# rdd0582/mri_superresolution

Measured on AMD Instinct MI355X. Metric: 2D MRI slices/sec (train fwd+bwd) 256×256 U-Net; PSNR/SSIM vs ref, higher is better.
Workload: dtype bf16; 1 GPU; UNetSuperRes base_filters=64 depth=4, 256x256 slices -> 512x512, batch=16/GPU bf16, L1+SSIM(0.4), train step fwd+bwd+Adam+SSIM metric; global_batch=16, parallelism=dp1

## Files before the change

include/mrisr.h:

```cpp
#ifndef MRISR_H
#define MRISR_H

#include <stddef.h>
#include <stdint.h>

#ifdef __cplusplus
extern "C" {
#endif

#define MRISR_OK 0
#define MRISR_E_ARG (-1)
#define MRISR_E_SHAPE (-2)
#define MRISR_E_DTYPE (-3)
#define MRISR_E_HIP (-4)
#define MRISR_E_UNSUPPORTED (-5)

#define MRISR_F32 0
#define MRISR_BF16 1
#define MRISR_F16 2

#define MRISR_SRC_RAW 0
#define MRISR_SRC_NORM 1
#define MRISR_SRC_RELU 2
#define MRISR_SP_NONE 0
// ... 112 lines not shown
                         const float* blend_alpha, void* g, float* red, float* alpha_slots, int N, int H, int W,
                         int C, int groups, void* stream);
int mrisr_act_bwd_finalize(const float* red, const float* gamma, const float* meanrstd, float* dgamma,
                           float* dbeta, float* coef, int N, int C, int groups, double count,
                           const float* alpha_slots, const float* alpha, float* dalpha, float alpha_sign, void* stream);
int mrisr_act_bwd_apply(int dtype, const void* x, const void* g, const float* coef, void* dx, int N,
                        int H, int W, int C, int out_mode, float* dbias, void* stream);
typedef struct mrisr_gn_bwd_fin {
    const float* red;
    const float* gamma;
    const float* meanrstd;
    float* dgamma;
    float* dbeta;
    const float* alpha_slots;
    const float* alpha;
    float* dalpha;
    double count;
    float alpha_sign;
    int32_t groups;
} mrisr_gn_bwd_fin;
int mrisr_act_bwd_apply_fused(int dtype, const void* x, const float* scale, const float* shift, int nconsumers,
                              const mrisr_consumer* consumers, const float* blend_alpha, const float* coef,
                              const mrisr_gn_bwd_fin* fin, void* dx, int N, int H, int W, int C, void* stream);
int mrisr_act_bwd_onepass_slots(void);
int mrisr_act_bwd_onepass_barrier_words(void);
int mrisr_act_bwd_onepass_ok(int dtype, int nconsumers, const mrisr_consumer* consumers, int N, int H, int W, int C);
int mrisr_act_bwd_onepass(int dtype, const void* x, const float* scale, const float* shift, const float* meanrstd,
                          int nconsumers, const mrisr_consumer* consumers, float* red, uint32_t* arrive,
                          const mrisr_gn_bwd_fin* fin, void* dx, int N, int H, int W, int C, void* stream);
int mrisr_act_bwd_apply_fused_unshuffle(int dtype, const void* x, const float* scale, const float* shift,
                                        const mrisr_consumer* consumer, const float* blend_alpha,
                                        const mrisr_gn_bwd_fin* fin, void* dx, float* dbias, int N, int H, int W, int C,
                                        void* stream);
int mrisr_channel_sum(int dtype, const void* x, float* out, size_t npix, int C, void* stream);
int mrisr_blend_alpha_grad(int dtype, const void* da, const void* x0, const float* scale0,
                           const float* shift0, const void* x1, const float* scale1,
                           const float* shift1, const float* alpha, float* dalpha, int N, int H,
                           int W, int C, void* stream);

int mrisr_head_forward(int dtype, const void* x, const float* scale, const float* shift,
                       const float* w, const float* b, float* out, int N, int H, int W, int C,
                       void* stream);
int mrisr_head_backward(int dtype, const void* x, const float* scale, const float* shift,
                        const float* w, const float* out, const float* dout, void* da, float* dw,
                        float* db, int N, int H, int W, int C, void* stream);
int mrisr_head_forward_multi(int dtype, const void* x, const float* scale, const float* shift,
                             const float* w, const float* b, float* out, int N, int H, int W, int C,
                             int K, void* stream);
int mrisr_head_backward_multi(int dtype, const void* x, const float* scale, const float* shift,
                              const float* w, const float* out, const float* dout, void* da,
                              float* dw, float* db, int N, int H, int W, int C, int K, void* stream);

int mrisr_ssim_l1_forward(const float* a, const float* b, double* sums, float* coef, int N, int H,
                          int W, float val_range, float sigma, void* stream);
int mrisr_ssim_l1_backward(const float* a, const float* b, const float* coef, const double* sums,
                           const float* gscale, float l1_w, float ssim_w, float* da, int N, int H,
                           int W, float sigma, void* stream);
int mrisr_ssim_l1_forward_win(const float* a, const float* b, double* sums, float* coef, int N, int H, int W,
                              float val_range, float sigma, int window_size, void* stream);
int mrisr_ssim_l1_backward_win(const float* a, const float* b, const float* coef, const double* sums,
                               const float* gscale, float l1_w, float ssim_w, float* da, int N, int H, int W,
                               float sigma, int window_size, void* stream);

int mrisr_loss_finalize(const double* sums, int N, int H, int W, float l1_w, float ssim_w, float* out,
                        void* stream);

// ... 89 lines not shown
```

mri_superresolution_amd/_lib.py:

```python
from __future__ import annotations

import ctypes as C
import os

from .tuning import TUNING

_HERE = os.path.dirname(os.path.abspath(__file__))
LIB_PATH = TUNING.lib_path or os.path.join(_HERE, "libmrisr.so")

F32, BF16, F16 = 0, 1, 2
SRC_RAW, SRC_NORM, SRC_RELU = 0, 1, 2
SP_NONE, SP_POOL2, SP_UP2, SP_HEAD = 0, 1, 2, 3
COMBINE_CONCAT, COMBINE_BLEND = 0, 1
OUT_PLAIN, OUT_PIXEL_SHUFFLE2 = 0, 1
UP2_BILINEAR, UP2_BICUBIC, UP2_SHARP_BILINEAR = 0, 1, 2
WINDOW_F32, WINDOW_I16 = 0, 1
RESAMPLE_LINEAR, RESAMPLE_CUBIC, RESAMPLE_AREA, RESAMPLE_LANCZOS4 = 1, 2, 3, 4
PACK_RING = 256
PACK_UPADJ = 512
STAT_SLOTS = 16

_vp, _fp, _dp, _i, _f, _d, _sz = C.c_void_p, C.c_void_p, C.c_void_p, C.c_int, C.c_float, C.c_double, C.c_size_t


class Src(C.Structure):
    _fields_ = [("ptr", _vp), ("scale", _fp), ("shift", _fp), ("C", C.c_int32), ("H", C.c_int32),
                ("W", C.c_int32), ("mode", C.c_int32), ("spatial", C.c_int32), ("off_y", C.c_int32),
                ("off_x", C.c_int32)]


class ConvDesc(C.Structure):
    _fields_ = [("dtype", C.c_int32), ("N", C.c_int32), ("H", C.c_int32), ("W", C.c_int32),
                ("Cin", C.c_int32), ("Cout", C.c_int32), ("ksize", C.c_int32), ("nsrc", C.c_int32),
                ("combine", C.c_int32), ("out_mode", C.c_int32), ("groups", C.c_int32),
                ("relu_out", C.c_int32), ("src", Src * 2), ("blend_alpha", _fp), ("wpacked", _vp),
                ("bias", _fp), ("out", _vp), ("stats", _dp), ("relu_mask", _vp), ("cu_limit", C.c_int32),
                ("reserved_", C.c_int32), ("wpacked_ring", _vp)]


class PackJob(C.Structure):
    _fields_ = [("w", _fp), ("packed", _vp), ("Cout", C.c_int32), ("Cin", C.c_int32), ("ksize", C.c_int32),
                ("transpose_flip", C.c_int32)]


class AugGeo(C.Structure):
    _fields_ = [("cos_a", C.c_float), ("sin_a", C.c_float), ("rotate", C.c_int32), ("flip", C.c_int32),
                ("fill", C.c_int32), ("brightness", C.c_float)]


class AugPhoto(C.Structure):
    _fields_ = [("contrast", C.c_float), ("mean", C.c_int32), ("noise_sigma", C.c_float), ("seed", C.c_uint32)]


class GnBwdFin(C.Structure):
    _fields_ = [("red", _fp), ("gamma", _fp), ("meanrstd", _fp), ("dgamma", _fp), ("dbeta", _fp),
                ("alpha_slots", _fp), ("alpha", _fp), ("dalpha", _fp), ("count", C.c_double),
                ("alpha_sign", C.c_float), ("groups", C.c_int32)]


class Consumer(C.Structure):
    _fields_ = [("da", _vp), ("C_total", C.c_int32), ("c_off", C.c_int32), ("H", C.c_int32),
                ("W", C.c_int32), ("spatial", C.c_int32), ("off_y", C.c_int32), ("off_x", C.c_int32),
                ("weight_mode", C.c_int32), ("head_out", _fp), ("head_w", _fp), ("head_part", _fp),
                ("head_dw", _fp), ("head_db", _fp)]


SIGNATURES = {
    "mrisr_last_error": (C.c_char_p, []),
    "mrisr_version": (_i, []),
    "mrisr_stat_slots": (_i, []),
    "mrisr_packed_weight_bytes": (_sz, [_i, _i, _i, _i]),
    "mrisr_conv_ring_bn": (_i, [_i, _i, _i, _i]),
    "mrisr_packed_weight_bytes_ring": (_sz, [_i, _i, _i, _i]),
    "mrisr_pack_weights": (_i, [_i, _fp, _i, _i, _i, _i, _vp, _vp]),
    "mrisr_pack_weights_batched": (_i, [_i, _vp, _i, _vp]),
    "mrisr_conv_forward": (_i, [C.POINTER(ConvDesc), _vp]),
    "mrisr_packed_weight_bytes_upadj": (_sz, [_i, _i, _i, _i]),
    "mrisr_conv_upadj": (_i, [C.POINTER(ConvDesc), _vp, _vp, _vp]),
    "mrisr_conv_variant": (_i, [C.POINTER(ConvDesc), _i, C.c_char_p, _sz]),
    "mrisr_conv_wgrad": (_i, [C.POINTER(ConvDesc), _vp, _fp, _fp, _sz, _vp]),
    "mrisr_conv_wgrad_workspace_floats": (_sz, [C.POINTER(ConvDesc)]),
    "mrisr_stem_forward": (_i, [_i, _fp, _fp, _vp, _dp, _i, _i, _i, _i, _i, _vp]),
    "mrisr_stem_wgrad": (_i, [_i, _fp, _vp, _fp, _i, _i, _i, _i, _vp]),
    "mrisr_stem_forward_multi": (_i, [_i, _fp, _fp, _vp, _dp, _i, _i, _i, _i, _i, _i, _vp]),
    "mrisr_stem_wgrad_multi": (_i, [_i, _fp, _vp, _fp, _i, _i, _i, _i, _i, _vp]),
    "mrisr_gn_finalize": (_i, [_dp, _fp, _fp, _fp, _fp, _fp, _i, _i, _i, _d, _f, _vp]),
    "mrisr_norm_pool2": (_i, [_i, _vp, _fp, _fp, _vp, _i, _i, _i, _i, _vp]),
    "mrisr_norm_upsample2": (_i, [_i, _vp, _fp, _fp, _vp, _i, _i, _i, _i, _vp]),
    "mrisr_norm_blend": (_i, [_i, _vp, _fp, _fp, _vp, _fp, _fp, _fp, _vp, _i, _i, _i, _i, _vp]),
    "mrisr_upsample2_stats": (_i, [_i, _vp, _vp, _dp, _i, _i, _i, _i, _i, _vp]),
    "mrisr_up_conv1x1_fused": (_i, [_i, _vp, _fp, _fp, _vp, _vp, _dp, _i, _i, _i, _i, _i, _i, _vp]),
    "mrisr_upsample2_adjoint": (_i, [_i, _vp, _vp, _i, _i, _i, _i, _vp]),
    "mrisr_act_bwd_reduce": (_i, [_i, _vp, _fp, _fp, _fp, _i, C.POINTER(Consumer), _fp, _vp, _fp, _fp, _i, _i, _i, _i, _i, _vp]),
    "mrisr_act_bwd_finalize": (_i, [_fp, _fp, _fp, _fp, _fp, _fp, _i, _i, _i, _d, _fp, _fp, _fp, _f, _vp]),
    "mrisr_act_bwd_apply": (_i, [_i, _vp, _vp, _fp, _vp, _i, _i, _i, _i, _i, _fp, _vp]),
    "mrisr_act_bwd_apply_fused": (_i, [_i, _vp, _fp, _fp, _i, C.POINTER(Consumer), _fp, _fp, C.POINTER(GnBwdFin), _vp, _i, _i,
                                       _i, _i, _vp]),
    "mrisr_act_bwd_onepass_slots": (_i, []),
    "mrisr_act_bwd_onepass_barrier_words": (_i, []),
    "mrisr_act_bwd_onepass_ok": (_i, [_i, _i, C.POINTER(Consumer), _i, _i, _i, _i]),
    "mrisr_act_bwd_onepass": (_i, [_i, _vp, _fp, _fp, _fp, _i, C.POINTER(Consumer), _fp, _vp, C.POINTER(GnBwdFin), _vp, _i, _i, _i,
                                   _i, _vp]),
    "mrisr_act_bwd_apply_fused_unshuffle": (_i, [_i, _vp, _fp, _fp, C.POINTER(Consumer), _fp, C.POINTER(GnBwdFin), _vp, _fp, _i,
                                                 _i, _i, _i, _vp]),
    "mrisr_channel_sum": (_i, [_i, _vp, _fp, _sz, _i, _vp]),
    "mrisr_blend_alpha_grad": (_i, [_i, _vp, _vp, _fp, _fp, _vp, _fp, _fp, _fp, _fp, _i, _i, _i, _i, _vp]),
    "mrisr_head_forward": (_i, [_i, _vp, _fp, _fp, _fp, _fp, _fp, _i, _i, _i, _i, _vp]),
    "mrisr_head_backward": (_i, [_i, _vp, _fp, _fp, _fp, _fp, _fp, _vp, _fp, _fp, _i, _i, _i, _i, _vp]),
    "mrisr_head_forward_multi": (_i, [_i, _vp, _fp, _fp, _fp, _fp, _fp, _i, _i, _i, _i, _i, _vp]),
    "mrisr_head_backward_multi": (_i, [_i, _vp, _fp, _fp, _fp, _fp, _fp, _vp, _fp, _fp, _i, _i, _i, _i, _i, _vp]),
    "mrisr_ssim_l1_forward": (_i, [_fp, _fp, _dp, _fp, _i, _i, _i, _f, _f, _vp]),
    "mrisr_ssim_l1_backward": (_i, [_fp, _fp, _fp, _dp, _fp, _f, _f, _fp, _i, _i, _i, _f, _vp]),
    "mrisr_ssim_l1_forward_win": (_i, [_fp, _fp, _dp, _fp, _i, _i, _i, _f, _f, _i, _vp]),
    "mrisr_ssim_l1_backward_win": (_i, [_fp, _fp, _fp, _dp, _fp, _f, _f, _fp, _i, _i, _i, _f, _i, _vp]),
    "mrisr_loss_finalize": (_i, [_dp, _i, _i, _i, _f, _f, _fp, _vp]),
    "mrisr_image_metrics": (_i, [_fp, _fp, _dp, _i, _i, _i, _f, _f, _i, _vp]),
    "mrisr_metrics_finalize": (_i, [_dp, _i, _i, _i, _f, _dp, _vp]),
    "mrisr_vgg_input_channels": (_i, []),
    "mrisr_vgg_input_forward": (_i, [_i, _fp, _vp, _sz, _vp]),
    "mrisr_vgg_input_backward": (_i, [_i, _vp, _fp, _f, _fp, _sz, _vp]),
    "mrisr_maxpool2_forward": (_i, [_i, _vp, _vp, _i, _i, _i, _i, _vp]),
    "mrisr_maxpool2_backward": (_i, [_i, _vp, _vp, _vp, _i, _i, _i, _i, _i, _vp]),
    "mrisr_feature_loss": (_i, [_i, _vp, _vp, _sz, _i, _dp, _fp, _vp, _i, _vp]),
    "mrisr_adam_step": (_i, [_fp, _fp, _fp, _fp, _sz, _f, _f, _f, _f, _f, _i, _f, _vp]),
    "mrisr_adam_step_amp": (_i, [_fp, _fp, _fp, _fp, _sz, _f, _f, _f, _f, _f, _vp, _f, _fp, _fp, _vp]),
    "mrisr_u8_histogram": (_i, [_vp, _sz, _i, _vp, _vp]),
    "mrisr_u8_percentile_normalise": (_i, [_vp, _vp, _sz, _i, _d, _d, _fp, _fp, _vp]),
    "mrisr_f32_to_u8": (_i, [_fp, _vp, _sz, _vp]),
    "mrisr_u8_upscale2": (_i, [_vp, _vp, _fp, _i, _i, _i, _i, _vp]),
    "mrisr_u8_to_unit_f32": (_i, [_vp, _fp, _sz, _vp]),
    "mrisr_augment_geo_u8": (_i, [_vp, _vp, _i, _i, _i, _vp, _dp, _vp]),
    "mrisr_augment_finish_u8": (_i, [_vp, _fp, _i, _sz, _vp, _dp, _vp]),
    "mrisr_cast": (_i, [_i, _vp, _i, _vp, _sz, _vp]),
    "mrisr_lowfield_dirichlet": (_i, [_i, _d, _fp, _fp]),
    "mrisr_lowfield_workspace_bytes": (_sz, [_i, _i, _i]),
    "mrisr_lowfield_simulate": (_i, [_vp, _i, _i, _i, _d, _fp, _fp, _fp, _fp, _f, _fp, _fp, _vp, _vp, _vp, _fp, _vp]),
    "mrisr_lowfield_dirichlet_any": (_i, [_i, _d, _fp, _fp]),
    "mrisr_lowfield_simulate_f32": (_i, [_fp, _i, _i, _i, _d, _fp, _fp, _fp, _fp, _f, _fp, _fp, _vp, _vp, _fp, _vp]),
    "mrisr_resample_taps": (_i, [_i, _i, _i, _i, _vp, _vp, _fp]),
    "mrisr_f32_resample_letterbox": (_i, [_fp, _i, _i, _i, _vp, _fp, _i, _i, _vp, _fp, _i, _i, _i, _i, _i, _i, _f, _i, _fp, _vp, _vp]),
    "mrisr_f32_percentile_workspace_bytes": (_sz, [_i]),
    "mrisr_f32_percentile_bounds": (_i, [_fp, _sz, _i, _d, _d, _fp, _vp, _vp]),
    "mrisr_f32_window_normalise": (_i, [_fp, _fp, _sz, _i, _fp, _vp]),
    "mrisr_f32_window_restore": (_i, [_fp, _fp, _sz, _i, _i, _vp, _vp]),
}

_lib = None
ABI_VERSION = 308


def load():
    global _lib
    if _lib is not None:
        return _lib
    if not os.path.exists(LIB_PATH):
        raise RuntimeError(
            f"{LIB_PATH} not found: the HIP kernel library is not built. Run "
            "`python -m mri_superresolution_amd.build` (needs hipcc); there is no CPU fallback.")
    lib = C.CDLL(LIB_PATH)
    missing = [name for name in SIGNATURES if not hasattr(lib, name)]
    if missing:
        raise RuntimeError(f"{LIB_PATH} lacks {len(missing)} symbol(s) of include/mrisr.h ({', '.join(missing[:4])}...): "
                           "header/library drift - rebuild with `python -m mri_superresolution_amd.build`")
    for name, (res, args) in SIGNATURES.items():
        fn = getattr(lib, name)
        fn.restype = res
        fn.argtypes = args
    if int(lib.mrisr_version()) != ABI_VERSION:
        raise RuntimeError(f"{LIB_PATH} is version {int(lib.mrisr_version())}, these bindings need {ABI_VERSION} (struct layouts "
                           "changed): rebuild with `python -m mri_superresolution_amd.build`")
    global STAT_SLOTS
    STAT_SLOTS = int(lib.mrisr_stat_slots())
    _lib = lib
    return lib


def check(rc: int, what: str = ""):
    if rc != 0:
        msg = load().mrisr_last_error().decode("utf-8", "replace")
        raise RuntimeError(f"libmrisr {what} failed ({rc}): {msg}")

# ... 38 lines not shown
```

mri_superresolution_amd/csrc/api.cpp:

```cpp
#include "common.h"
thread_local char g_mrisr_err[512] = "";
extern "C" const char* mrisr_last_error(void) { return g_mrisr_err; }
extern "C" int mrisr_version(void) { return 308; }
extern "C" int mrisr_stat_slots(void) { return MRISR_STAT_SLOTS; }
```

mri_superresolution_amd/csrc/norm.hip:

```cpp
#include "common.h"

__global__ void gn_finalize_kernel(const double* __restrict__ stats, const float* __restrict__ gamma,
                                   const float* __restrict__ beta, float* __restrict__ scale,
                                   float* __restrict__ shift, float* __restrict__ meanrstd, int N, int C,
                                   int groups, double count, float eps) {
    const int idx = blockIdx.x * blockDim.x + threadIdx.x;
    if (idx >= N * C) return;
    const int n = idx / C, c = idx - n * C;
    const int gs = C / groups, g = c / gs;
    typedef __attribute__((ext_vector_type(2))) double f64x2;
    f64x2 v[MRISR_STAT_SLOTS];
#pragma unroll
    for (int k = 0; k < MRISR_STAT_SLOTS; ++k) v[k] = *reinterpret_cast<const f64x2*>(stats + ((size_t)(k * N + n) * groups + g) * 2);
    double s = 0.0, ss = 0.0;
#pragma unroll
    for (int k = 0; k < MRISR_STAT_SLOTS; ++k) { s += v[k][0]; ss += v[k][1]; }
    const double mean = s / count;
    double var = ss / count - mean * mean;
    if (var < 0) var = 0;
    const float rstd = (float)(1.0 / sqrt(var + (double)eps));
    const float m = (float)mean;
    const float sc = gamma[c] * rstd;
    scale[idx] = sc;
    shift[idx] = beta[c] - m * sc;
// ... 1179 lines not shown
                                                   const mrisr_gn_bwd_fin* fin, void* dx, float* dbias, int N, int H, int W,
                                                   int C, void* stream) {
    if (!x || !scale || !shift || !dx || !consumer || !fin) MRISR_FAIL(MRISR_E_ARG, "act_bwd_apply_fused_unshuffle: null pointer");
    if (!fin->red || !fin->gamma || !fin->meanrstd || !fin->dgamma || !fin->dbeta) MRISR_FAIL(MRISR_E_ARG, "act_bwd_apply_fused_unshuffle: fin null pointer");
    if (fin->groups <= 0 || fin->groups > kMaxGroups || C % fin->groups || !(fin->count > 0)) MRISR_FAIL(MRISR_E_SHAPE, "act_bwd_apply_fused_unshuffle: fin groups %d", fin->groups);
    if (fin->alpha_slots && (!fin->alpha || !fin->dalpha)) MRISR_FAIL(MRISR_E_ARG, "act_bwd_apply_fused_unshuffle: alpha_slots without alpha/dalpha");
    const int vec = mrisr_vec(dtype);
    if (C % vec || ((H | W) & 1)) MRISR_FAIL(MRISR_E_SHAPE, "act_bwd_apply_fused_unshuffle: C %d, H %d, W %d (even dims)", C, H, W);
    if (consumer->spatial != MRISR_SP_NONE || consumer->H != H || consumer->W != W || consumer->off_y || consumer->off_x)
        MRISR_FAIL(MRISR_E_UNSUPPORTED, "act_bwd_apply_fused_unshuffle: one plain consumer with the node's geometry");
    ActBwdParams p;
    memset(&p, 0, sizeof(p));
    p.x = x; p.scale = scale; p.shift = shift; p.blend_alpha = blend_alpha;
    p.ncons = 1; p.N = N; p.H = H; p.W = W; p.C = C;
    int rc = fill_act_bwd_params(p, dtype, 1, consumer, blend_alpha, H, W, C, "act_bwd_apply_fused_unshuffle");
    if (rc) return rc;
    const FinDev fd{fin->red, fin->gamma, fin->meanrstd, fin->dgamma, fin->dbeta, fin->alpha_slots, fin->alpha, fin->dalpha,
                    (float)(1.0 / fin->count), fin->alpha_sign, fin->groups, nullptr, nullptr, nullptr};
    const int nslice = ceil_div(C / vec, 256), nvs = nslice > 1 ? 256 : C / vec;
    const int ppbw = 256 / nvs, HWp = (H / 2) * (W / 2);
    int ppw = ppbw * 16;
    if (ppw > HWp) ppw = ceil_div(HWp, ppbw) * ppbw;
    p.pix_per_block = ppw;
    dim3 grid(ceil_div(HWp, ppw), N, nslice);
    hipStream_t s = (hipStream_t)stream;
    if (dtype == MRISR_BF16) act_bwd_unshuffle_window_kernel<bf16_t><<<grid, 256, 0, s>>>(p, (bf16_t*)dx, dbias, fd);
    else if (dtype == MRISR_F16) act_bwd_unshuffle_window_kernel<f16_t><<<grid, 256, 0, s>>>(p, (f16_t*)dx, dbias, fd);
    else if (dtype == MRISR_F32) act_bwd_unshuffle_window_kernel<float><<<grid, 256, 0, s>>>(p, (float*)dx, dbias, fd);
    else MRISR_FAIL(MRISR_E_DTYPE, "act_bwd_apply_fused_unshuffle: dtype %d", dtype);
    MRISR_CHECK_LAUNCH("act_bwd_apply_fused_unshuffle");
    return MRISR_OK;
}

extern "C" int mrisr_act_bwd_apply(int dtype, const void* x, const void* g, const float* coef, void* dx, int N, int H,
                                   int W, int C, int out_mode, float* dbias, void* stream) {
    if (!x || !g || !coef || !dx) MRISR_FAIL(MRISR_E_ARG, "act_bwd_apply: null pointer");
    const int vec = mrisr_vec(dtype);
    if (C % vec) MRISR_FAIL(MRISR_E_SHAPE, "act_bwd_apply: C %d", C);
    if (out_mode == MRISR_OUT_PIXEL_SHUFFLE2 && ((H | W) & 1)) MRISR_FAIL(MRISR_E_SHAPE, "act_bwd_apply: odd dims with pixel shuffle");
    const size_t total = (size_t)N * H * W * (C / vec);
    const int blocks = (int)((total + 255) / 256 < 8192 ? (total + 255) / 256 : 8192);
    if (dbias && !(out_mode == MRISR_OUT_PIXEL_SHUFFLE2 && (4 * C) % vec == 0 && 256 % (4 * C / vec) == 0))
        MRISR_FAIL(MRISR_E_UNSUPPORTED, "act_bwd_apply: dbias needs the pixel-shuffle output with 4C/vec dividing 256");
    if (out_mode == MRISR_OUT_PIXEL_SHUFFLE2 && (4 * C) % vec == 0) {
        const int blocks = dbias ? (int)((total + 255) / 256 < 1024 ? (total + 255) / 256 : 1024) : (int)((total + 255) / 256 < 8192 ? (total + 255) / 256 : 8192);
        if (dtype == MRISR_BF16)
            act_bwd_apply_unshuffle_kernel<bf16_t><<<blocks, 256, 0, (hipStream_t)stream>>>((const bf16_t*)x, (const bf16_t*)g, coef, (bf16_t*)dx, N, H, W, C, dbias);
        else if (dtype == MRISR_F16)
            act_bwd_apply_unshuffle_kernel<f16_t><<<blocks, 256, 0, (hipStream_t)stream>>>((const f16_t*)x, (const f16_t*)g, coef, (f16_t*)dx, N, H, W, C, dbias);
        else if (dtype == MRISR_F32)
            act_bwd_apply_unshuffle_kernel<float><<<blocks, 256, 0, (hipStream_t)stream>>>((const float*)x, (const float*)g, coef, (float*)dx, N, H, W, C, dbias);
        else MRISR_FAIL(MRISR_E_DTYPE, "act_bwd_apply: dtype %d", dtype);
        MRISR_CHECK_LAUNCH("act_bwd_apply");
        return MRISR_OK;
    }
    if (dtype == MRISR_BF16)
        act_bwd_apply_kernel<bf16_t><<<blocks, 256, 0, (hipStream_t)stream>>>((const bf16_t*)x, (const bf16_t*)g, coef, (bf16_t*)dx, N, H, W, C, out_mode);
    else if (dtype == MRISR_F16)
        act_bwd_apply_kernel<f16_t><<<blocks, 256, 0, (hipStream_t)stream>>>((const f16_t*)x, (const f16_t*)g, coef, (f16_t*)dx, N, H, W, C, out_mode);
    else if (dtype == MRISR_F32)
        act_bwd_apply_kernel<float><<<blocks, 256, 0, (hipStream_t)stream>>>((const float*)x, (const float*)g, coef, (float*)dx, N, H, W, C, out_mode);
    else MRISR_FAIL(MRISR_E_DTYPE, "act_bwd_apply: dtype %d", dtype);
    MRISR_CHECK_LAUNCH("act_bwd_apply");
    return MRISR_OK;
}

// ... 475 lines not shown
```

mri_superresolution_amd/engine.py:

```python
from __future__ import annotations

import ctypes as C
from dataclasses import dataclass
from typing import Dict, List, Optional, Tuple

import torch

from . import _lib as L
from .launch import GN_GROUPS, Consumer, dgrad_desc, gn_finalize, marshal_consumers
from .tuning import TUNING


def _dt(dtype: torch.dtype) -> int:
    if dtype == torch.bfloat16:
        return L.BF16
    if dtype == torch.float16:
        return L.F16
    if dtype == torch.float32:
        return L.F32
    raise ValueError(f"unsupported compute dtype {dtype} (use torch.float32, torch.float16 or torch.bfloat16)")


@dataclass(frozen=True, eq=False)
class Node:
# ... 107 lines not shown

        def dconv(prefix, src: Tuple[Source, ...], cin, cout, combine=L.COMBINE_CONCAT, pool_src=False):
            a = node(f"{prefix}.double_conv.0", cout, f"{prefix}.double_conv.1.weight", f"{prefix}.double_conv.1.bias")
            self.layers.append(Layer(f"{prefix}.double_conv.0", cin, cout, 3, src, a, combine, pool_src=pool_src))
            b = node(f"{prefix}.double_conv.3", cout, f"{prefix}.double_conv.4.weight", f"{prefix}.double_conv.4.bias")
            self.layers.append(Layer(f"{prefix}.double_conv.3", cout, cout, 3, (Source(a),), b))
            return b

        self.stem = node("inc.double_conv.0", f, "inc.double_conv.1.weight", "inc.double_conv.1.bias")
        x1 = node("inc.double_conv.3", f, "inc.double_conv.4.weight", "inc.double_conv.4.bias")
        self.layers.append(Layer("inc.double_conv.3", f, f, 3, (Source(self.stem),), x1))
        if depth < 2:
            raise ValueError("depth must be >= 2")
        self.depth = depth
        xs = [x1]
        for k in range(1, depth):
            xs.append(dconv(f"down{k}.maxpool_conv.1", (Source(xs[-1]),), f * 2 ** (k - 1), f * 2 ** k, pool_src=True))
        u = xs[-1]
        for j in range(1, depth):
            skip, cout = xs[depth - 1 - j], f * 2 ** (depth - 1 - j)
            up = node(f"up{j}.up.1", cout, f"up{j}.up.2.weight", f"up{j}.up.2.bias")
            self.layers.append(Layer(f"up{j}.up.1", 2 * cout, cout, 1, (Source(u),), up, post_up=True))
            u = dconv(f"up{j}.conv", (Source(skip), Source(up)), 2 * cout, cout)
        fb = node("final_up_bilinear.1", f // 2, "final_up_bilinear.2.weight", "final_up_bilinear.2.bias")
        self.layers.append(Layer("final_up_bilinear.1", f, f // 2, 3, (Source(u),), fb, up_src=True))
        ps = node("final_up_pixelshuffle.conv", f // 2, "final_up_pixelshuffle.norm.weight",
                  "final_up_pixelshuffle.norm.bias", shuffled=True)
        self.layers.append(Layer("final_up_pixelshuffle.conv", f, 2 * f, 3, (Source(u),), ps, bias=True,
                                 out_mode=L.OUT_PIXEL_SHUFFLE2))
        fc = node("final_conv.0", f // 2, "final_conv.1.weight", "final_conv.1.bias")
        self.layers.append(Layer("final_conv.0", f // 2, f // 2, 3, (Source(fb), Source(ps)), fc,
                                 combine=L.COMBINE_BLEND, blend_src=True))
        self.head_in = fc
        self._packed: Dict[tuple, torch.Tensor] = {}
        self._packed_token = None
        self.timer: Optional[KernelTimer] = None

    def _launch(self, kind, desc, fn):
        if self.timer is None:
            return fn()
        flops = 2.0 * desc.N * desc.H * desc.W * desc.Cin * desc.Cout * desc.ksize * desc.ksize
        if kind == "upadj":
            flops /= 4
        buf = C.create_string_buffer(96)
        L.call("mrisr_conv_variant", C.byref(desc), {"wgrad": 1, "upadj": 2}.get(kind, 0), buf, 96)
        self.timer.launch(buf.value.decode(), flops, fn)

    def _packed_buf(self, layer: Layer, w, dt: int, flip: int, ring: bool = False, upadj: bool = False):
        key = (layer.name, dt, "upadj") if upadj else (layer.name, dt, flip, "ring") if ring else (layer.name, dt, flip)
        buf = self._packed.get(key)
        if buf is None or buf.device != w.device:
            if upadj:
                nbytes = L.load().mrisr_packed_weight_bytes_upadj(dt, layer.cout, layer.cin, layer.ks)
            else:
                size = L.load().mrisr_packed_weight_bytes_ring if ring else L.load().mrisr_packed_weight_bytes
                nbytes = size(dt, layer.cin if flip else layer.cout, layer.cout if flip else layer.cin, layer.ks)
            buf = torch.empty(nbytes, dtype=torch.uint8, device=w.device)
            self._packed[key] = buf
        return buf

    def invalidate_packed(self):
        self._packed.clear()
        self._jobs_key = None
        self._packed_token = None

    def _pack_all(self, params, dt: int, stream, token=None):
# ... 152 lines not shown
            if layer.post_up:
                L.call("mrisr_upsample2_stats", dt, zlow.data_ptr(), o.raw.data_ptr(), o.stats.data_ptr(),
                       N, vh, vw, oC, GN_GROUPS, st, nbytes=N * vh * vw * oC * es * 5)
            finalize(layer.out)

        hn, hC = ns[self.head_in], self.head_in.C
        p.out = torch.empty((N, self.cout, hn.H, hn.W), dtype=torch.float32, device=dev)
        L.call("mrisr_head_forward_multi", dt, hn.raw.data_ptr(), hn.scale.data_ptr(), hn.shift.data_ptr(),
               params["final_conv.3.weight"].data_ptr(), params["final_conv.3.bias"].data_ptr(), p.out.data_ptr(),
               N, hn.H, hn.W, hC, self.cout, st, nbytes=N * hn.H * hn.W * (hC * es + 4 * self.cout))
        return p.out, (p if training else None)

    def backward(self, params, grads, ctx: _Pass, dout: torch.Tensor, bucket_hook=None):
        dtype = ctx.dtype
        dt = _dt(dtype)
        es = 4 if dtype == torch.float32 else 2
        N = ctx.N
        x = ctx.x
        dev = x.device
        st = L.stream_ptr()
        ns, ls = ctx.nodes, ctx.layers
        dout = dout.contiguous()

        narr = N * L.load().mrisr_act_bwd_onepass_barrier_words()
        SL = L.load().mrisr_act_bwd_onepass_slots() if es == 2 else 1
        red_sizes = [SL * N * n.C * 2 + 256 + narr + (N * (n.C + 1) if n is self.head_in else 0) for n in self.nodes.values()]
        red_arena = torch.zeros(sum(red_sizes), dtype=torch.float32, device=dev)
        red_off = {}
        o = 0
        for n, sz in zip(self.nodes.values(), red_sizes):
            red_off[n] = (o, sz)
            o += sz

        def node_backward(n: Node, dbias=None) -> torch.Tensor:
            s = ns[n]
            H, W, Cn = s.H, s.W, n.C
            consumers = s.consumers
            s.consumers = []
            cons = marshal_consumers(consumers)
            ncons = len(consumers)
            c0 = consumers[0]
            own = all((c.H, c.W, c.off_y, c.off_x) == (H, W, 0, 0) for c in consumers if c.spatial == L.SP_NONE)
            plain = all(c.spatial in (L.SP_NONE, L.SP_HEAD) for c in consumers)
            window = (not plain and H % 2 == 0 and W % 2 == 0 and own
                      and sum(c.spatial == L.SP_POOL2 for c in consumers) == 1
                      and all(c.spatial in (L.SP_POOL2, L.SP_NONE) for c in consumers))
            fused = (not n.shuffled) and (plain or window)
            fused_ps = n.shuffled and ncons == 1 and c0.spatial == L.SP_NONE and H % 2 == 0 and W % 2 == 0 and own
            uses_alpha = any(c.weight_mode != 0 for c in consumers)
            alpha_ptr = params["alpha"].data_ptr() if uses_alpha else None
            red = red_arena[red_off[n][0]:red_off[n][0] + red_off[n][1]]
            blend_branch = c0.weight_mode != 0 and c0.spatial == L.SP_NONE
            slots = red[SL * N * Cn * 2:] if blend_branch else None
            alpha_sign = 1.0 if c0.weight_mode == 1 else -1.0
            nx = N * H * W * Cn * es
            nda = sum(N * c.H * c.W * (8 if c.spatial == L.SP_HEAD else Cn * es) for c in consumers)
            count = float((Cn // GN_GROUPS) * H * W)
            dalpha_ptr = grads["alpha"].data_ptr() if slots is not None else None
            gn = (red.data_ptr(), params[n.gamma].data_ptr(), s.meanrstd.data_ptr(), grads[n.gamma].data_ptr(),
                  grads[n.beta].data_ptr())

            def onepass():
                arrive = red[SL * N * Cn * 2 + 256:SL * N * Cn * 2 + 256 + narr]
                f = L.GnBwdFin(*gn, None, None, None, count, 1.0, GN_GROUPS)
                dx = torch.empty_like(s.raw)
                L.call("mrisr_act_bwd_onepass", dt, s.raw.data_ptr(), s.scale.data_ptr(), s.shift.data_ptr(),
                       s.meanrstd.data_ptr(), ncons, cons, red.data_ptr(), arrive.data_ptr(), C.byref(f),
# ... 5 lines not shown
                       s.meanrstd.data_ptr(), ncons, cons, alpha_ptr, L.ptr(g), red.data_ptr(), L.ptr(slots),
                       N, H, W, Cn, GN_GROUPS, st, nbytes=nx + nda + (nx if g is not None else 0))

            def fused_unshuffle():
                f = L.GnBwdFin(*gn, L.ptr(slots), alpha_ptr, dalpha_ptr, count, alpha_sign, GN_GROUPS)
                dx = torch.empty((N, H // 2, W // 2, 4 * Cn), dtype=dtype, device=dev)
                L.call("mrisr_act_bwd_apply_fused_unshuffle", dt, s.raw.data_ptr(), s.scale.data_ptr(),
                       s.shift.data_ptr(), cons, alpha_ptr, C.byref(f), dx.data_ptr(), L.ptr(dbias), N, H, W, Cn, st,
                       nbytes=2 * nx + nda)
                return dx

            def fused_apply():
                f = L.GnBwdFin(*gn, L.ptr(slots), alpha_ptr, dalpha_ptr, count, alpha_sign, GN_GROUPS)
                dx = torch.empty_like(s.raw)
                L.call("mrisr_act_bwd_apply_fused", dt, s.raw.data_ptr(), s.scale.data_ptr(), s.shift.data_ptr(),
                       ncons, cons, alpha_ptr, None, C.byref(f), dx.data_ptr(), N, H, W, Cn, st,
                       nbytes=2 * nx + nda)
                return dx

            def general(g):
                coef = torch.empty(3 * N * Cn, dtype=torch.float32, device=dev)
                L.call("mrisr_act_bwd_finalize", *gn, coef.data_ptr(), N, Cn, GN_GROUPS, count, L.ptr(slots), alpha_ptr, dalpha_ptr,
                       alpha_sign, st)
                if n.shuffled:
                    dx = torch.empty((N, H // 2, W // 2, 4 * Cn), dtype=dtype, device=dev)
                    mode = L.OUT_PIXEL_SHUFFLE2
                else:
                    dx = torch.empty_like(s.raw)
                    mode = L.OUT_PLAIN
                L.call("mrisr_act_bwd_apply", dt, s.raw.data_ptr(), g.data_ptr(), coef.data_ptr(), dx.data_ptr(),
                       N, H, W, Cn, mode, L.ptr(dbias) if n.shuffled else None, st, nbytes=3 * nx)
                return dx

            op_blocks = -(-(H * W) // ((256 // max(Cn // 8, 1)) * 8)) if Cn >= 8 else 1 << 30
            if (fused and slots is None and not uses_alpha
                    and op_blocks <= (128 if bucket_hook is not None else 256)
                    and L.load().mrisr_act_bwd_onepass_ok(dt, ncons, cons, N, H, W, Cn)):
                return onepass()
            g = None if (fused or fused_ps) else torch.empty_like(s.raw)
            reduce(g)
            if fused_ps:
                return fused_unshuffle()
            if fused:
                return fused_apply()
            return general(g)

        hn, hC = ns[self.head_in], self.head_in.C
        ho = red_off[self.head_in][0] + SL * N * hC * 2 + 256 + narr
        if self.cout == 1:
            hn.consumers.append(Consumer(dout, hC, 0, hn.H, hn.W, L.SP_HEAD, 0, 0, head=(
                ctx.out, params["final_conv.3.weight"], red_arena[ho:ho + N * (hC + 1)], grads["final_conv.3.weight"],
                grads["final_conv.3.bias"])))
        else:
            dah = torch.empty_like(hn.raw)
            L.call("mrisr_head_backward_multi", dt, hn.raw.data_ptr(), hn.scale.data_ptr(), hn.shift.data_ptr(),
                   params["final_conv.3.weight"].data_ptr(), ctx.out.data_ptr(), dout.data_ptr(), dah.data_ptr(),
                   grads["final_conv.3.weight"].data_ptr(), grads["final_conv.3.bias"].data_ptr(), N, hn.H, hn.W, hC,
                   self.cout, st, nbytes=N * hn.H * hn.W * (2 * hC * es + 8 * self.cout))
            hn.consumers.append(Consumer(dah, hC, 0, hn.H, hn.W, L.SP_NONE, 0, 0))

        side = None
        main = torch.cuda.current_stream()
        side_default = L.num_cus() * 13 // 32 if self.f <= 64 else L.num_cus() * 3 // 8
        side_cus = side_default if TUNING.wgrad_cus < 0 else TUNING.wgrad_cus
        if TUNING.wgrad_stream and self.timer is None:
            side = getattr(self, "_side_stream", None)
# ... 89 lines not shown
```

Before: 2079 slices/s.

## Fuse GroupNorm backward for both blend branches into paired reduce/apply kernels

Adds paired reduce and apply kernels that process the pixel-shuffle branch and the bilinear branch of the final blend together. Each kernel reads the shared upstream gradient once instead of once per branch, and the per-branch reduce/apply launches collapse into two launches. The sibling's result is cached so its later node_backward call returns it directly. This adds larger register footprints (waves_per_eu pinned to 2) and more complex eligibility checks, plus ordering assumptions about when the sibling's consumers are ready.

Result: faster. 2118 slices/s, median of 6 (+1.9%).

```diff
diff --git a/include/mrisr.h b/include/mrisr.h
--- a/include/mrisr.h
+++ b/include/mrisr.h
@@ -168,6 +168,22 @@
                                         const mrisr_consumer* consumer, const float* blend_alpha,
                                         const mrisr_gn_bwd_fin* fin, void* dx, float* dbias, int N, int H, int W, int C,
                                         void* stream);
+typedef struct mrisr_blend_branch {
+    const void* x;
+    const float* scale;
+    const float* shift;
+    const float* meanrstd;
+    float* red;
+    float* alpha_slots;
+    int32_t weight_mode;
+    int32_t reserved_;
+} mrisr_blend_branch;
+int mrisr_act_bwd_blend_ok(int dtype, int N, int H, int W, int C);
+int mrisr_act_bwd_blend_reduce(int dtype, const void* da, const mrisr_blend_branch* ps, const mrisr_blend_branch* bil,
+                               const float* blend_alpha, int N, int H, int W, int C, int groups, void* stream);
+int mrisr_act_bwd_blend_apply(int dtype, const void* da, const mrisr_blend_branch* ps, const mrisr_blend_branch* bil,
+                              const float* blend_alpha, const mrisr_gn_bwd_fin* fin_ps, const mrisr_gn_bwd_fin* fin_bil,
+                              void* dx_ps, void* dx_bil, float* dbias, int N, int H, int W, int C, void* stream);
 int mrisr_channel_sum(int dtype, const void* x, float* out, size_t npix, int C, void* stream);
 int mrisr_blend_alpha_grad(int dtype, const void* da, const void* x0, const float* scale0,
                            const float* shift0, const void* x1, const float* scale1,
diff --git a/mri_superresolution_amd/_lib.py b/mri_superresolution_amd/_lib.py
--- a/mri_superresolution_amd/_lib.py
+++ b/mri_superresolution_amd/_lib.py
@@ -56,6 +56,11 @@
     _fields_ = [("red", _fp), ("gamma", _fp), ("meanrstd", _fp), ("dgamma", _fp), ("dbeta", _fp),
                 ("alpha_slots", _fp), ("alpha", _fp), ("dalpha", _fp), ("count", C.c_double),
                 ("alpha_sign", C.c_float), ("groups", C.c_int32)]
+
+
+class BlendBranch(C.Structure):
+    _fields_ = [("x", _vp), ("scale", _fp), ("shift", _fp), ("meanrstd", _fp), ("red", _fp), ("alpha_slots", _fp),
+                ("weight_mode", C.c_int32), ("reserved_", C.c_int32)]
 
 
 class Consumer(C.Structure):
@@ -103,6 +108,10 @@
                                    _i, _vp]),
     "mrisr_act_bwd_apply_fused_unshuffle": (_i, [_i, _vp, _fp, _fp, C.POINTER(Consumer), _fp, C.POINTER(GnBwdFin), _vp, _fp, _i,
                                                  _i, _i, _i, _vp]),
+    "mrisr_act_bwd_blend_ok": (_i, [_i, _i, _i, _i, _i]),
+    "mrisr_act_bwd_blend_reduce": (_i, [_i, _vp, C.POINTER(BlendBranch), C.POINTER(BlendBranch), _fp, _i, _i, _i, _i, _i, _vp]),
+    "mrisr_act_bwd_blend_apply": (_i, [_i, _vp, C.POINTER(BlendBranch), C.POINTER(BlendBranch), _fp, C.POINTER(GnBwdFin),
+                                       C.POINTER(GnBwdFin), _vp, _vp, _fp, _i, _i, _i, _i, _vp]),
     "mrisr_channel_sum": (_i, [_i, _vp, _fp, _sz, _i, _vp]),
     "mrisr_blend_alpha_grad": (_i, [_i, _vp, _vp, _fp, _fp, _vp, _fp, _fp, _fp, _fp, _i, _i, _i, _i, _vp]),
     "mrisr_head_forward": (_i, [_i, _vp, _fp, _fp, _fp, _fp, _fp, _i, _i, _i, _i, _vp]),
@@ -146,7 +155,7 @@
 }
 
 _lib = None
-ABI_VERSION = 308
+ABI_VERSION = 309
 
 
 def load():
diff --git a/mri_superresolution_amd/csrc/api.cpp b/mri_superresolution_amd/csrc/api.cpp
--- a/mri_superresolution_amd/csrc/api.cpp
+++ b/mri_superresolution_amd/csrc/api.cpp
@@ -1,5 +1,5 @@
 #include "common.h"
 thread_local char g_mrisr_err[512] = "";
 extern "C" const char* mrisr_last_error(void) { return g_mrisr_err; }
-extern "C" int mrisr_version(void) { return 308; }
+extern "C" int mrisr_version(void) { return 309; }
 extern "C" int mrisr_stat_slots(void) { return MRISR_STAT_SLOTS; }
diff --git a/mri_superresolution_amd/csrc/norm.hip b/mri_superresolution_amd/csrc/norm.hip
--- a/mri_superresolution_amd/csrc/norm.hip
+++ b/mri_superresolution_amd/csrc/norm.hip
@@ -1235,6 +1235,278 @@
     return MRISR_OK;
 }
 
+struct BlendBranchDev {
+    const void* x;
+    const float* scale;
+    const float* shift;
+    const float* meanrstd;
+    float* red;
+    float* alpha_slots;
+    int weight_mode;
+};
+struct BlendBwdParams {
+    const void* da;
+    const float* blend_alpha;
+    BlendBranchDev br[2];
+    int N, H, W, C, groups, pix_per_block;
+};
+
+template <typename T>
+__global__ __launch_bounds__(256) __attribute__((amdgpu_waves_per_eu(2, 2))) void act_bwd_blend_reduce_kernel(const BlendBwdParams p) {
+    constexpr int VEC = Vec16<T>::N;
+    __shared__ float lds[256 * VEC * 2];
+    const int t = threadIdx.x, n = blockIdx.y;
+    const int nvec = p.C / VEC, ppb = 256 / nvec;
+    const int cv = t % nvec, pl = t / nvec, c = cv * VEC;
+    const bool active = pl < ppb;
+    const int Wp = p.W / 2, HWp = (p.H / 2) * Wp, W = p.W;
+    const int gs = p.C / p.groups;
+    const float a = 1.f / (1.f + __expf(-p.blend_alpha[0]));
+    float wgt[2], sc[2][VEC], sh[2][VEC], sA[2][VEC], sB[2][VEC], adot[2] = {0.f, 0.f};
+    const T* xb[2];
+#pragma unroll
+    for (int b = 0; b < 2; ++b) {
+        wgt[b] = p.br[b].weight_mode == 1 ? a : 1.f - a;
+        xb[b] = (const T*)p.br[b].x + (size_t)n * p.H * W * p.C + c;
+#pragma unroll
+        for (int e = 0; e < VEC; ++e) {
+            sc[b][e] = p.br[b].scale[(size_t)n * p.C + c + e];
+            sh[b][e] = p.br[b].shift[(size_t)n * p.C + c + e];
+            sA[b][e] = 0.f;
+            sB[b][e] = 0.f;
+        }
+    }
+    const T* db = (const T*)p.da + (size_t)n * p.H * W * p.C + c;
+    const int pend = min(HWp, (int)(blockIdx.x + 1) * p.pix_per_block);
+    if (active) {
+#pragma unroll 1
+        for (int pp = blockIdx.x * p.pix_per_block + pl; pp < pend; pp += ppb) {
+            const int py = pp / Wp, px = pp - py * Wp;
+            const size_t b0 = (size_t)(2 * py) * W + 2 * px;
+#pragma unroll
+            for (int r = 0; r < 2; ++r) {
+                const size_t o0 = b0 + (size_t)r * W;
+                Vec16<T> dv[2], xv[2][2];
+#pragma unroll
+                for (int q = 0; q < 2; ++q) {
+                    dv[q] = load_vec16(db + (o0 + q) * p.C);
+                    xv[0][q] = load_vec16(xb[0] + (o0 + q) * p.C);
+                    xv[1][q] = load_vec16(xb[1] + (o0 + q) * p.C);
+                }
+#pragma unroll
+                for (int q = 0; q < 2; ++q) {
+#pragma unroll
+                    for (int e = 0; e < VEC; ++e) {
+                        const float d = dv[q].get(e);
+#pragma unroll
+                        for (int b = 0; b < 2; ++b) {
+                            const float xr = xv[b][q].get(e);
+                            const float pre = xr * sc[b][e] + sh[b][e];
+                            const float gy = wgt[b] * d * (pre > 0.f ? 1.f : LRELU_SLOPE);
+                            sA[b][e] += gy;
+                            sB[b][e] += gy * xr;
+                            adot[b] += d * lrelu(pre);
+                        }
+                    }
+                }
+            }
+        }
+    }
+#pragma unroll
+    for (int b = 0; b < 2; ++b) {
+        const BlendBranchDev& br = p.br[b];
+#pragma unroll
+        for (int e = 0; e < VEC; ++e) {
+            const int g = (c + e) / gs;
+            const float mean = br.meanrstd[((size_t)n * p.groups + g) * 2], rstd = br.meanrstd[((size_t)n * p.groups + g) * 2 + 1];
+            sB[b][e] = rstd * (sB[b][e] - mean * sA[b][e]);
+        }
+        const float w = wave_sum(active ? adot[b] : 0.f);
+        if ((t & 63) == 0) atomic_add_f32(&br.alpha_slots[(blockIdx.x * 4 + (t >> 6) + blockIdx.y * 37) & 255], w);
+        if (b) __syncthreads();
+#pragma unroll
+        for (int e = 0; e < VEC; ++e) {
+            lds[(t * VEC + e) * 2] = active ? sA[b][e] : 0.f;
+            lds[(t * VEC + e) * 2 + 1] = active ? sB[b][e] : 0.f;
+        }
+        __syncthreads();
+        for (int i = t; i < nvec * VEC * 2; i += 256) {
+            const int j = i >> 1, which = i & 1;
+            const int cvj = j / VEC, e = j - cvj * VEC;
+            float s = 0.f;
+            for (int q = 0; q < ppb; ++q) s += lds[((q * nvec + cvj) * VEC + e) * 2 + which];
+            atomic_add_f32(&br.red[((size_t)n * p.C + cvj * VEC + e) * 2 + which], s);
+        }
+    }
+}
+
+template <typename T>
+__global__ __launch_bounds__(256) __attribute__((amdgpu_waves_per_eu(2, 2))) void act_bwd_blend_apply_kernel(const BlendBwdParams p, T* __restrict__ dx_ps, T* __restrict__ dx_bil,
+                                                                  float* __restrict__ dbias, const FinDev fin_ps, const FinDev fin_bil) {
+    constexpr int VEC = Vec16<T>::N;
+    __shared__ float lds[256 * 4 * VEC];
+    const int t = threadIdx.x, n = blockIdx.y;
+    const int nvec = p.C / VEC, ppb = 256 / nvec;
+    const int cv = t % nvec, pl = t / nvec, c = cv * VEC;
+    const bool active = pl < ppb;
+    const int Wp = p.W / 2, HWp = (p.H / 2) * Wp, W = p.W;
+    float sc[2][VEC], sh[2][VEC], ca[2][VEC], cb[2][VEC], cc[2][VEC], bs[4 * VEC];
+    const bool owner = blockIdx.x == 0, first = blockIdx.x + blockIdx.y == 0;
+    gn_bwd_coefs<VEC>(fin_ps, lds, n, p.C, c, active, owner, pl == 0, first, ca[0], cb[0], cc[0]);
+    __syncthreads();
+    gn_bwd_coefs<VEC>(fin_bil, lds, n, p.C, c, active, owner, pl == 0, first, ca[1], cb[1], cc[1]);
+    const float a = 1.f / (1.f + __expf(-p.blend_alpha[0]));
+    float wgt[2];
+    const T* xb[2];
+    const size_t k0 = (size_t)n * p.C + c;
+#pragma unroll
+    for (int b = 0; b < 2; ++b) {
+        wgt[b] = p.br[b].weight_mode == 1 ? a : 1.f - a;
+        xb[b] = (const T*)p.br[b].x + (size_t)n * p.H * W * p.C + c;
+#pragma unroll
+        for (int e = 0; e < VEC; ++e) {
+            sc[b][e] = p.br[b].scale[k0 + e];
+            sh[b][e] = p.br[b].shift[k0 + e];
+        }
+    }
+#pragma unroll
+    for (int i = 0; i < 4 * VEC; ++i) bs[i] = 0.f;
+    const T* db = (const T*)p.da + (size_t)n * p.H * W * p.C + c;
+    T* ops = dx_ps + (size_t)n * HWp * 4 * p.C + 4 * c;
+    T* obl = dx_bil + (size_t)n * p.H * W * p.C + c;
+    const int pend = min(HWp, (int)(blockIdx.x + 1) * p.pix_per_block);
+    if (active) {
+        for (int pp = blockIdx.x * p.pix_per_block + pl; pp < pend; pp += ppb) {
+            const int py = pp / Wp, px = pp - py * Wp;
+            const size_t b0 = (size_t)(2 * py) * W + 2 * px;
+            const size_t off[4] = {b0, b0 + 1, b0 + W, b0 + W + 1};
+            Vec16<T> dv[4], xv[4], yv[4];
+#pragma unroll
+            for (int q = 0; q < 4; ++q) {
+                dv[q] = load_vec16(db + off[q] * p.C);
+                xv[q] = load_vec16(xb[0] + off[q] * p.C);
+                yv[q] = load_vec16(xb[1] + off[q] * p.C);
+            }
+            Vec16<T> ov[4];
+#pragma unroll
+            for (int e = 0; e < VEC; ++e) {
+#pragma unroll
+                for (int q = 0; q < 4; ++q) {
+                    const float xr = xv[q].get(e);
+                    const float pre = xr * sc[0][e] + sh[0][e];
+                    const float gy = wgt[0] * dv[q].get(e) * (pre > 0.f ? 1.f : LRELU_SLOPE);
+                    const int i = 4 * e + q;
+                    ov[i / VEC].set(i % VEC, gy * ca[0][e] + xr * cb[0][e] + cc[0][e]);
+                }
+            }
+#pragma unroll
+            for (int j = 0; j < 4; ++j) store_vec16(ops + (size_t)pp * 4 * p.C + j * VEC, ov[j]);
+            if (dbias) {
+#pragma unroll
+                for (int i = 0; i < 4 * VEC; ++i) bs[i] += ov[i / VEC].get(i % VEC);
+            }
+#pragma unroll
+            for (int q = 0; q < 4; ++q) {
+                Vec16<T> o;
+#pragma unroll
+                for (int e = 0; e < VEC; ++e) {
+                    const float xr = yv[q].get(e);
+                    const float pre = xr * sc[1][e] + sh[1][e];
+                    const float gy = wgt[1] * dv[q].get(e) * (pre > 0.f ? 1.f : LRELU_SLOPE);
+                    o.set(e, gy * ca[1][e] + xr * cb[1][e] + cc[1][e]);
+                }
+                store_vec16(obl + off[q] * p.C, o);
+            }
+        }
+    }
+    if (dbias) {
+        __syncthreads();
+#pragma unroll
+        for (int i = 0; i < 4 * VEC; ++i) lds[t * 4 * VEC + i] = active ? bs[i] : 0.f;
+        __syncthreads();
+        for (int j = t; j < nvec * 4 * VEC; j += 256) {
+            const int cvj = j / (4 * VEC), i = j - cvj * 4 * VEC;
+            float v = 0.f;
+            for (int q = 0; q < ppb; ++q) v += lds[(q * nvec + cvj) * 4 * VEC + i];
+            atomic_add_f32(&dbias[4 * cvj * VEC + i], v);
+        }
+    }
+}
+
+extern "C" int mrisr_act_bwd_blend_ok(int dtype, int N, int H, int W, int C) {
+    if (dtype != MRISR_BF16 && dtype != MRISR_F16) return 0;
+    if (N < 1 || N > 65535 || H < 2 || W < 2 || ((H | W) & 1) || C < 1) return 0;
+    const int vec = mrisr_vec(dtype);
+    if (C % vec || C / vec > 256) return 0;
+    if ((long)H * W >= (1l << 31)) return 0;
+    return 1;
+}
+
+static int fill_blend_params(BlendBwdParams& p, int dtype, const void* da, const mrisr_blend_branch* ps, const mrisr_blend_branch* bil,
+                             const float* blend_alpha, int N, int H, int W, int C, int groups, const char* who) {
+    if (!da || !ps || !bil || !blend_alpha) MRISR_FAIL(MRISR_E_ARG, "%s: null pointer", who);
+    if (!mrisr_act_bwd_blend_ok(dtype, N, H, W, C)) MRISR_FAIL(MRISR_E_UNSUPPORTED, "%s: shape does not qualify (mrisr_act_bwd_blend_ok)", who);
+    if (groups <= 0 || groups > kMaxGroups || C % groups) MRISR_FAIL(MRISR_E_SHAPE, "%s: C %d groups %d", who, C, groups);
+    memset(&p, 0, sizeof(p));
+    p.da = da; p.blend_alpha = blend_alpha;
+    p.N = N; p.H = H; p.W = W; p.C = C; p.groups = groups;
+    const mrisr_blend_branch* src[2] = {ps, bil};
+    for (int b = 0; b < 2; ++b) {
+        const mrisr_blend_branch& s = *src[b];
+        if (!s.x || !s.scale || !s.shift || !s.meanrstd || !s.red || !s.alpha_slots) MRISR_FAIL(MRISR_E_ARG, "%s: branch %d null pointer", who, b);
+        if (s.weight_mode != 1 && s.weight_mode != 2) MRISR_FAIL(MRISR_E_ARG, "%s: branch %d weight_mode", who, b);
+        p.br[b] = BlendBranchDev{s.x, s.scale, s.shift, s.meanrstd, s.red, s.alpha_slots, s.weight_mode};
+    }
+    return MRISR_OK;
+}
+
+extern "C" int mrisr_act_bwd_blend_reduce(int dtype, const void* da, const mrisr_blend_branch* ps, const mrisr_blend_branch* bil,
+                                          const float* blend_alpha, int N, int H, int W, int C, int groups, void* stream) {
+    BlendBwdParams p;
+    int rc = fill_blend_params(p, dtype, da, ps, bil, blend_alpha, N, H, W, C, groups, "act_bwd_blend_reduce");
+    if (rc) return rc;
+    const int ppb = 256 / (C / mrisr_vec(dtype)), HWp = (H / 2) * (W / 2);
+    int ppw = ppb * 8;
+    if (ppw > HWp) ppw = ceil_div(HWp, ppb) * ppb;
+    p.pix_per_block = ppw;
+    dim3 grid(ceil_div(HWp, ppw), N);
+    hipStream_t s = (hipStream_t)stream;
+    if (dtype == MRISR_BF16) act_bwd_blend_reduce_kernel<bf16_t><<<grid, 256, 0, s>>>(p);
+    else act_bwd_blend_reduce_kernel<f16_t><<<grid, 256, 0, s>>>(p);
+    MRISR_CHECK_LAUNCH("act_bwd_blend_reduce");
+    return MRISR_OK;
+}
+
+extern "C" int mrisr_act_bwd_blend_apply(int dtype, const void* da, const mrisr_blend_branch* ps, const mrisr_blend_branch* bil,
+                                         const float* blend_alpha, const mrisr_gn_bwd_fin* fin_ps, const mrisr_gn_bwd_fin* fin_bil,
+                                         void* dx_ps, void* dx_bil, float* dbias, int N, int H, int W, int C, void* stream) {
+    if (!fin_ps || !fin_bil || !dx_ps || !dx_bil) MRISR_FAIL(MRISR_E_ARG, "act_bwd_blend_apply: null pointer");
+    if (fin_ps->groups != fin_bil->groups) MRISR_FAIL(MRISR_E_SHAPE, "act_bwd_blend_apply: fin groups %d and %d", fin_ps->groups, fin_bil->groups);
+    BlendBwdParams p;
+    int rc = fill_blend_params(p, dtype, da, ps, bil, blend_alpha, N, H, W, C, fin_ps->groups, "act_bwd_blend_apply");
+    if (rc) return rc;
+    const mrisr_gn_bwd_fin* fins[2] = {fin_ps, fin_bil};
+    FinDev fd[2];
+    for (int b = 0; b < 2; ++b) {
+        const mrisr_gn_bwd_fin* f = fins[b];
+        if (f->red != p.br[b].red || !f->gamma || !f->meanrstd || !f->dgamma || !f->dbeta) MRISR_FAIL(MRISR_E_ARG, "act_bwd_blend_apply: fin %d", b);
+        if (!(f->count > 0)) MRISR_FAIL(MRISR_E_SHAPE, "act_bwd_blend_apply: fin %d count", b);
+        if (f->alpha_slots != p.br[b].alpha_slots || !f->alpha || !f->dalpha) MRISR_FAIL(MRISR_E_ARG, "act_bwd_blend_apply: fin %d alpha_slots / alpha / dalpha", b);
+        fd[b] = FinDev{f->red, f->gamma, f->meanrstd, f->dgamma, f->dbeta, f->alpha_slots, f->alpha, f->dalpha,
+                       (float)(1.0 / f->count), f->alpha_sign, f->groups, nullptr, nullptr, nullptr};
+    }
+    const int ppb = 256 / (C / mrisr_vec(dtype)), HWp = (H / 2) * (W / 2);
+    int ppw = ppb * 16;
+    if (ppw > HWp) ppw = ceil_div(HWp, ppb) * ppb;
+    p.pix_per_block = ppw;
+    dim3 grid(ceil_div(HWp, ppw), N);
+    hipStream_t s = (hipStream_t)stream;
+    if (dtype == MRISR_BF16) act_bwd_blend_apply_kernel<bf16_t><<<grid, 256, 0, s>>>(p, (bf16_t*)dx_ps, (bf16_t*)dx_bil, dbias, fd[0], fd[1]);
+    else act_bwd_blend_apply_kernel<f16_t><<<grid, 256, 0, s>>>(p, (f16_t*)dx_ps, (f16_t*)dx_bil, dbias, fd[0], fd[1]);
+    MRISR_CHECK_LAUNCH("act_bwd_blend_apply");
+    return MRISR_OK;
+}
+
 extern "C" int mrisr_act_bwd_apply(int dtype, const void* x, const void* g, const float* coef, void* dx, int N, int H,
                                    int W, int C, int out_mode, float* dbias, void* stream) {
     if (!x || !g || !coef || !dx) MRISR_FAIL(MRISR_E_ARG, "act_bwd_apply: null pointer");
diff --git a/mri_superresolution_amd/engine.py b/mri_superresolution_amd/engine.py
--- a/mri_superresolution_amd/engine.py
+++ b/mri_superresolution_amd/engine.py
@@ -163,6 +163,11 @@
         self.layers.append(Layer("final_conv.0", f // 2, f // 2, 3, (Source(fb), Source(ps)), fc,
                                  combine=L.COMBINE_BLEND, blend_src=True))
         self.head_in = fc
+        self._blend_sibling: Dict[Node, Node] = {}
+        for layer in self.layers:
+            if layer.combine == L.COMBINE_BLEND:
+                a, b = (src.node for src in layer.srcs)
+                self._blend_sibling[a], self._blend_sibling[b] = b, a
         self._packed: Dict[tuple, torch.Tensor] = {}
         self._packed_token = None
         self.timer: Optional[KernelTimer] = None
@@ -381,7 +386,11 @@
             red_off[n] = (o, sz)
             o += sz
 
+        blend_dx: Dict[Node, torch.Tensor] = {}
+
         def node_backward(n: Node, dbias=None) -> torch.Tensor:
+            if n in blend_dx:
+                return blend_dx.pop(n)
             s = ns[n]
             H, W, Cn = s.H, s.W, n.C
             consumers = s.consumers
@@ -453,6 +462,42 @@
                        N, H, W, Cn, mode, L.ptr(dbias) if n.shuffled else None, st, nbytes=3 * nx)
                 return dx
 
+            def blend_pair():
+                sib = self._blend_sibling.get(n)
+                if sib is None or not (fused_ps and blend_branch) or sib.shuffled or sib.C != Cn or (c0.C_total, c0.c_off) != (Cn, 0):
+                    return None
+                t = ns[sib]
+                if len(t.consumers) != 1 or (t.H, t.W) != (H, W):
+                    return None
+                k = t.consumers[0]
+                if (k.da is not c0.da or k.weight_mode not in (1, 2) or k.weight_mode == c0.weight_mode or k.spatial != L.SP_NONE
+                        or (k.H, k.W, k.off_y, k.off_x, k.C_total, k.c_off) != (H, W, 0, 0, Cn, 0)):
+                    return None
+                if not L.load().mrisr_act_bwd_blend_ok(dt, N, H, W, Cn):
+                    return None
+                t.consumers = []
+                red_s = red_arena[red_off[sib][0]:red_off[sib][0] + red_off[sib][1]]
+                slots_s = red_s[SL * N * Cn * 2:]
+                bp = L.BlendBranch(s.raw.data_ptr(), s.scale.data_ptr(), s.shift.data_ptr(), s.meanrstd.data_ptr(), red.data_ptr(),
+                                   slots.data_ptr(), c0.weight_mode, 0)
+                bb = L.BlendBranch(t.raw.data_ptr(), t.scale.data_ptr(), t.shift.data_ptr(), t.meanrstd.data_ptr(), red_s.data_ptr(),
+                                   slots_s.data_ptr(), k.weight_mode, 0)
+                L.call("mrisr_act_bwd_blend_reduce", dt, c0.da.data_ptr(), C.byref(bp), C.byref(bb), alpha_ptr, N, H, W, Cn,
+                       GN_GROUPS, st, nbytes=3 * nx)
+                fp = L.GnBwdFin(*gn, slots.data_ptr(), alpha_ptr, dalpha_ptr, count, alpha_sign, GN_GROUPS)
+                fb = L.GnBwdFin(red_s.data_ptr(), params[sib.gamma].data_ptr(), t.meanrstd.data_ptr(), grads[sib.gamma].data_ptr(),
+                                grads[sib.beta].data_ptr(), slots_s.data_ptr(), alpha_ptr, dalpha_ptr, count,
+                                1.0 if k.weight_mode == 1 else -1.0, GN_GROUPS)
+                dx = torch.empty((N, H // 2, W // 2, 4 * Cn), dtype=dtype, device=dev)
+                dx_sib = torch.empty_like(t.raw)
+                L.call("mrisr_act_bwd_blend_apply", dt, c0.da.data_ptr(), C.byref(bp), C.byref(bb), alpha_ptr, C.byref(fp),
+                       C.byref(fb), dx.data_ptr(), dx_sib.data_ptr(), L.ptr(dbias), N, H, W, Cn, st, nbytes=5 * nx)
+                blend_dx[sib] = dx_sib
+                return dx
+
+            dx = blend_pair()
+            if dx is not None:
+                return dx
             op_blocks = -(-(H * W) // ((256 // max(Cn // 8, 1)) * 8)) if Cn >= 8 else 1 << 30
             if (fused and slots is None and not uses_alpha
                     and op_blocks <= (128 if bucket_hook is not None else 256)
```
